# TORlN/HDR-to-SDR

Hardware: AMD Instinct MI355X
Metric: Mpixel/s HDR10->SDR (4K frames) at 1/2/4/8 GPUs; % HBM roofline (higher is better)
Workload: dtype f32

## Files before the change

### hdr-to-sdr_amd/csrc/h2s_tile.h

```cpp
#pragma once
#include <hip/hip_runtime.h>

#include <type_traits>

#include "h2s_device.h"
#include "h2s_dovi.h"

#ifndef H2S_TAGSEL
#define H2S_TAGSEL 1
#endif
#ifndef H2S_EQMAGIC
#define H2S_EQMAGIC 1
#endif
#ifdef H2S_ISA_MARKS
#define H2S_MARK(name)                  \
  do {                                  \
    __builtin_amdgcn_sched_barrier(0);  \
    asm volatile(";@@" name);           \
    __builtin_amdgcn_sched_barrier(0);  \
  } while (0)
#define H2S_MARKV(name, a, b, c)                                  \
  do {                                                            \
    __builtin_amdgcn_sched_barrier(0);                            \
    asm volatile(";@@" name : "+v"(a), "+v"(b), "+v"(c));         \
// ... 577 lines not shown
    asm("v_lshlrev_b16 %0, 1, %1" : "=v"(off) : "v"(qb));
    return *reinterpret_cast<const uint16_t*>(reinterpret_cast<const char*>(eq_lds) + off);
  } else {
    return eq_lds[(int)o.x];
  }
}

constexpr int CBW = 32, CBH = 16;
#ifndef H2S_YST
#define H2S_YST 72
#endif
#ifndef H2S_YST_LP
#define H2S_YST_LP 68
#endif
template <int LP>
constexpr int row_stride() { return LP ? H2S_YST_LP : H2S_YST; }
#ifndef H2S_NT_LOAD
#define H2S_NT_LOAD 2
#endif
#ifndef H2S_NT_STORE
#define H2S_NT_STORE 2
#endif
constexpr int NT = H2S_NT_LOAD, NTS = H2S_NT_STORE;

__device__ __forceinline__ float quad_sum(float v) {
  v += __builtin_bit_cast(float, __builtin_amdgcn_update_dpp(0, __builtin_bit_cast(int, v), 0xB1, 0xF, 0xF, false));
  return v + __builtin_bit_cast(float, __builtin_amdgcn_update_dpp(0, __builtin_bit_cast(int, v), 0x4E, 0xF, 0xF, false));
}

__device__ __forceinline__ void unpack8(const uint4 a, float* o) {
  o[0] = (float)(a.x & 0xffff), o[1] = (float)(a.x >> 16), o[2] = (float)(a.y & 0xffff), o[3] = (float)(a.y >> 16);
  o[4] = (float)(a.z & 0xffff), o[5] = (float)(a.z >> 16), o[6] = (float)(a.w & 0xffff), o[7] = (float)(a.w >> 16);
}

template <class T>
__device__ __forceinline__ T in_vgpr(T x) {
  T y;
  asm volatile("v_mov_b32 %0, %1" : "=v"(y) : "s"(x));
  return y;
}

__device__ __forceinline__ __amdgpu_buffer_rsrc_t plane_rsrc(const uint8_t* base, int bytes) {
  return __builtin_amdgcn_make_buffer_rsrc((void*)base, (short)0, bytes, 0x00020000);
}

template <bool SEMI, int SUB = 0>
struct TileRegs {
  uint4 ya, ua;
  std::conditional_t<SEMI, unsigned, uint16_t> uh;
};
template <bool SEMI>
struct TileRegs<SEMI, 2> {
  uint4 ya, ua, va;
};

struct TileGeo {
  int f, px0, py0, cx0, cy0;
};

__device__ __forceinline__ CurveConsts curve_of(const CurveConsts* frames, int f) {
  typedef __attribute__((address_space(4))) const float cfloat;
  constexpr int n = (int)(sizeof(CurveConsts) / sizeof(float));
  cfloat* src = (cfloat*)frames + __builtin_amdgcn_readfirstlane(f) * n;
  CurveConsts r;
  float* dst = reinterpret_cast<float*>(&r);
#pragma unroll
  for (int i = 0; i < n; i++) dst[i] = src[i];
  return r;
}

__device__ __forceinline__ TileGeo tile_geo(const FastParams& F, unsigned tile) {
  const unsigned bx = tile % F.nbx, bt = tile / F.nbx;
  TileGeo g;
  g.f = (int)(bt / F.nby);
  const int by = (int)(bt % F.nby);
  g.px0 = (int)bx * TBW, g.py0 = by * TBH, g.cx0 = (int)bx * CBW, g.cy0 = by * CBH;
  return g;
}

__device__ __forceinline__ void tile_next(const FastParams& F, TileGeo& g) {
  g.px0 += TBW, g.cx0 += CBW;
  if (g.px0 >= F.W) {
    g.px0 = 0, g.cx0 = 0, g.py0 += TBH, g.cy0 += CBH;
    if (g.py0 >= (int)F.nby * TBH) g.py0 = 0, g.cy0 = 0, g.f++;
  }
}

struct LaneOfs {
  int y, u;
  int sy, sc;
};

template <bool SEMI>
__device__ __forceinline__ LaneOfs lane_ofs(const FastParams& F, int t) {
  LaneOfs L;
  L.y = (t >> 3) * (int)F.in_ls[0] + 16 * (t & 7);
  const int pc = (t >> 7) & 1, tc = t & 127;
  L.u = (tc >> 2) * (int)F.in_ls[1 + pc] + 16 * (tc & 3);
  if (SEMI && F.in_semi) L.u = (t >> 3) * (int)F.in_ls[1] + 16 * (t & 7);
  const int sb = F.out8 ? 8 : 16;
  L.sy = (t >> 3) * (int)F.out_ls[0] + sb * (t & 7);
  const int pl = (t >> 6) & 1, rem = t & 63;
  L.sc = (rem >> 2) * (int)F.out_ls[1 + pl] + sb * (rem & 3);
  if (SEMI && F.out_semi) L.sc = (t >> 3) * (int)F.out_ls[1] + sb * (t & 7);
  return L;
}

template <bool SEMI, int SUB = 0>
__device__ __forceinline__ TileRegs<SEMI, SUB> tile_load(const FastParams& F, const TileGeo& g, int t, const LaneOfs& L) {
  const __amdgpu_buffer_rsrc_t iy = plane_rsrc(F.in[0] + g.f * F.in_fp[0], F.in_bytes[0]);
  const int yr = t >> 3, yc = t & 7;
  TileRegs<SEMI, SUB> r;
  int vy, sy;
  if (g.py0 + TBH <= F.H) {
    vy = L.y, sy = g.py0 * (int)F.in_ls[0] + 2 * g.px0;
  } else {
    vy = (g.py0 + yr < F.H ? g.py0 + yr : F.H - 1) * (int)F.in_ls[0] + 2 * (g.px0 + 8 * yc), sy = 0;
  }
  r.ya = __builtin_bit_cast(uint4, __builtin_amdgcn_raw_buffer_load_b128(iy, vy, sy, NT));
  if constexpr (SUB == 2) {
    const __amdgpu_buffer_rsrc_t iu = plane_rsrc(F.in[1] + g.f * F.in_fp[1], F.in_bytes[1]);
    const __amdgpu_buffer_rsrc_t iv = plane_rsrc(F.in[2] + g.f * F.in_fp[2], F.in_bytes[2]);
    const int lu = (int)F.in_ls[1], lv = (int)F.in_ls[2];
    int vu, vv, su, sv;
    if (g.py0 + TBH <= F.H) {
      vu = yr * lu + 16 * yc, vv = yr * lv + 16 * yc;
      su = g.py0 * lu + 2 * g.px0, sv = g.py0 * lv + 2 * g.px0;
    } else {
      const int row = g.py0 + yr < F.H ? g.py0 + yr : F.H - 1;
      vu = row * lu + 2 * (g.px0 + 8 * yc), vv = row * lv + 2 * (g.px0 + 8 * yc), su = sv = 0;
    }
    r.ua = __builtin_bit_cast(uint4, __builtin_amdgcn_raw_buffer_load_b128(iu, vu, su, NT));
    r.va = __builtin_bit_cast(uint4, __builtin_amdgcn_raw_buffer_load_b128(iv, vv, sv, NT));
    return r;
  } else if constexpr (SUB == 1) {
    const int pc = __builtin_amdgcn_readfirstlane(t >> 7), tc = t & 127;
    const __amdgpu_buffer_rsrc_t ic = plane_rsrc(F.in[1 + pc] + g.f * F.in_fp[1 + pc], F.in_bytes[1 + pc]);
    const int ls = (int)F.in_ls[1 + pc];
    int vc, vh, sc;
    if (g.py0 + TBH <= F.H && g.cx0 + CBW + 1 <= F.icw) {
      vc = L.u, vh = L.u + 16, sc = g.py0 * ls + 2 * g.cx0;
    } else {
      const int clr = tc >> 2, ccx = tc & 3;
      const int row = g.py0 + clr < F.H ? g.py0 + clr : F.H - 1;
      vc = row * ls + 2 * (g.cx0 + 8 * ccx);
      vh = row * ls + 2 * chroma_edge_at(g.cx0 + 8 * ccx + 8, F.icw, F.chroma_edge);
      sc = 0;
    }
    if ((tc & 3) != 3) vh = 0x7FFFFFF0;
    r.ua = __builtin_bit_cast(uint4, __builtin_amdgcn_raw_buffer_load_b128(ic, vc, sc, NT));
    r.uh = __builtin_amdgcn_raw_buffer_load_b16(ic, vh, sc, 0);
    return r;
  } else {
  if (SEMI && F.in_semi) {
    const __amdgpu_buffer_rsrc_t ic = plane_rsrc(F.in[1] + g.f * F.in_fp[1], F.in_bytes[1]);
    const int ls = (int)F.in_ls[1];
    int vc, vh, sc;
    if (g.cy0 >= 1 && g.cy0 + CBH + 1 <= F.ch && g.cx0 + CBW + 1 <= F.cw) {
      vc = L.u, vh = L.u + 16, sc = (g.cy0 - 1) * ls + 4 * g.cx0;
    } else {
      const int clr = t >> 3, ccx = t & 7;
      const int row = chroma_edge_at(g.cy0 - 1 + clr, F.ch, F.chroma_edge);
      vc = row * ls + 4 * (g.cx0 + 4 * ccx);
      vh = row * ls + 4 * chroma_edge_at(g.cx0 + 4 * ccx + 4, F.cw, F.chroma_edge);
      sc = 0;
    }
    if (t >= 144) vc = vh = 0x7FFFFFF0;
    r.ua = __builtin_bit_cast(uint4, __builtin_amdgcn_raw_buffer_load_b128(ic, vc, sc, NT));
    r.uh = __builtin_amdgcn_raw_buffer_load_b32(ic, vh, sc, 0);
    return r;
  }
  const int pc = __builtin_amdgcn_readfirstlane(t >> 7), tc = t & 127;
  const __amdgpu_buffer_rsrc_t ic = plane_rsrc(F.in[1 + pc] + g.f * F.in_fp[1 + pc], F.in_bytes[1 + pc]);
  const int ls = (int)F.in_ls[1 + pc];
  int vc, vh, sc;
  if (g.cy0 >= 1 && g.cy0 + CBH + 1 <= F.ch && g.cx0 + CBW + 1 <= F.cw) {
    vc = L.u, vh = L.u + 16, sc = (g.cy0 - 1) * ls + 2 * g.cx0;
  } else {
    const int clr = tc >> 2, ccx = tc & 3;
    const int row = chroma_edge_at(g.cy0 - 1 + clr, F.ch, F.chroma_edge);
    vc = row * ls + 2 * (g.cx0 + 8 * ccx);
    vh = row * ls + 2 * chroma_edge_at(g.cx0 + 8 * ccx + 8, F.cw, F.chroma_edge);
    sc = 0;
  }
  if (tc >= 72) vc = vh = 0x7FFFFFF0;
  r.ua = __builtin_bit_cast(uint4, __builtin_amdgcn_raw_buffer_load_b128(ic, vc, sc, NT));
  r.uh = __builtin_amdgcn_raw_buffer_load_b16(ic, vh, sc, 0);
  return r;
  }
}

template <int YST>
__device__ __forceinline__ float stage_luma(float* yin, uint4 a, int row, int col8, float ysc, float yoff) {
  float v[8];
  unpack8(a, v);
  float* d = yin + row * YST + 8 * col8;
  const float4 lo = make_float4(fmaf(v[0], ysc, yoff), fmaf(v[1], ysc, yoff), fmaf(v[2], ysc, yoff), fmaf(v[3], ysc, yoff));
  const float4 hi = make_float4(fmaf(v[4], ysc, yoff), fmaf(v[5], ysc, yoff), fmaf(v[6], ysc, yoff), fmaf(v[7], ysc, yoff));
  *reinterpret_cast<float4*>(d) = lo;
  *reinterpret_cast<float4*>(d + 4) = hi;
  return __builtin_fmaxf(__builtin_fmaxf(__builtin_fmaxf(lo.x, lo.y), __builtin_fmaxf(lo.z, lo.w)),
                         __builtin_fmaxf(__builtin_fmaxf(hi.x, hi.y), __builtin_fmaxf(hi.z, hi.w)));
}
template <int HST>
__device__ __forceinline__ float stage_chroma(float* plane, uint4 a, unsigned h, int tt, float cmid) {
  float v[9];
  unpack8(a, v);
  v[8] = (float)h;
#pragma unroll
  for (int k = 0; k < 9; k++) v[k] -= cmid;
  float m = fabsf(v[0]);
#pragma unroll
  for (int k = 1; k < 9; k++) m = __builtin_fmaxf(m, fabsf(v[k]));
  float* d = plane + (tt >> 2) * HST + 16 * (tt & 3);
#pragma unroll
  for (int k = 0; k < 4; k++)
    *reinterpret_cast<float4*>(d + 4 * k) =
        make_float4(v[2 * k] + v[2 * k], v[2 * k] + v[2 * k + 1], v[2 * k + 1] + v[2 * k + 1], v[2 * k + 1] + v[2 * k + 2]);
  return m;
}
template <int HST>
__device__ __forceinline__ float stage_chroma_semi(float* plane_u, float* plane_v, uint4 a, unsigned h, int tt, float cmid) {
  const unsigned w[5] = {a.x, a.y, a.z, a.w, h};
  float u[5], v[5];
#pragma unroll
  for (int k = 0; k < 5; k++) u[k] = (float)(w[k] & 0xffff) - cmid, v[k] = (float)(w[k] >> 16) - cmid;
  float m = __builtin_fmaxf(fabsf(u[0]), fabsf(v[0]));
#pragma unroll
  for (int k = 1; k < 5; k++) m = __builtin_fmaxf(m, __builtin_fmaxf(fabsf(u[k]), fabsf(v[k])));
  const int o = (tt >> 3) * HST + 8 * (tt & 7);
#pragma unroll
  for (int k = 0; k < 2; k++) {
    *reinterpret_cast<float4*>(plane_u + o + 4 * k) =
        make_float4(u[2 * k] + u[2 * k], u[2 * k] + u[2 * k + 1], u[2 * k + 1] + u[2 * k + 1], u[2 * k + 1] + u[2 * k + 2]);
    *reinterpret_cast<float4*>(plane_v + o + 4 * k) =
        make_float4(v[2 * k] + v[2 * k], v[2 * k] + v[2 * k + 1], v[2 * k + 1] + v[2 * k + 1], v[2 * k + 1] + v[2 * k + 2]);
  }
  return m;
}
constexpr int C422_ST = 36;
constexpr int C444_ST = 72;
__device__ __forceinline__ float stage_chroma422(float* plane, uint4 a, unsigned h, int tt, float cmid) {
  float v[9];
  unpack8(a, v);
  v[8] = (float)h;
#pragma unroll
  for (int k = 0; k < 9; k++) v[k] -= cmid;
  float m = fabsf(v[0]);
#pragma unroll
  for (int k = 1; k < 8; k++) m = __builtin_fmaxf(m, fabsf(v[k]));
  float* d = plane + (tt >> 2) * C422_ST + 8 * (tt & 3);
  *reinterpret_cast<float4*>(d) = make_float4(v[0], v[1], v[2], v[3]);
  *reinterpret_cast<float4*>(d + 4) = make_float4(v[4], v[5], v[6], v[7]);
  if ((tt & 3) == 3) d[8] = v[8], m = __builtin_fmaxf(m, fabsf(v[8]));
  return m;
}
__device__ __forceinline__ float stage_chroma444(float* plane_u, float* plane_v, uint4 a, uint4 b, int row, int col8,
                                                 int imid) {
  auto pack = [&](uint4 q, float* plane, float& m) {
    const unsigned w[4] = {q.x, q.y, q.z, q.w};
    unsigned o[4];
#pragma unroll
    for (int k = 0; k < 4; k++) {
      const int lo = (int)(w[k] & 0xffff) - imid, hi = (int)(w[k] >> 16) - imid;
      m = __builtin_fmaxf(m, __builtin_fmaxf(fabsf((float)lo), fabsf((float)hi)));
      o[k] = ((unsigned)lo & 0xffffu) | ((unsigned)hi << 16);
    }
    *reinterpret_cast<uint4*>(reinterpret_cast<int16_t*>(plane) + row * C444_ST + 8 * col8) = make_uint4(o[0], o[1], o[2], o[3]);
  };
  float m = 0.0f;
  pack(a, plane_u, m);
  pack(b, plane_v, m);
  return m;
}
template <int YST>
__device__ __forceinline__ u4v read_luma(const FastParams& F, const float* yin, int r, int c) {
  const unsigned* src = reinterpret_cast<const unsigned*>(yin) + r * YST + 8 * c;
  const uint4 a = *reinterpret_cast<const uint4*>(src), b = *reinterpret_cast<const uint4*>(src + 4);
  if (F.out8)
    return u4v{a.x | (a.y << 8) | (a.z << 16) | (a.w << 24), b.x | (b.y << 8) | (b.z << 16) | (b.w << 24), 0u, 0u};
  return u4v{a.x | (a.y << 16), a.z | (a.w << 16), b.x | (b.y << 16), b.z | (b.w << 16)};
}
__device__ __forceinline__ void put_luma(const FastParams& F, const TileGeo& g, u4v v, int r, int vo, int so) {
  if (g.py0 + r >= F.H) return;
  const __amdgpu_buffer_rsrc_t oy_ = plane_rsrc(F.out[0] + g.f * F.out_fp[0], F.out_bytes[0]);
  so += g.py0 * (int)F.out_ls[0];
  if (F.out8)
    __builtin_amdgcn_raw_buffer_store_b64(u2v{v.x, v.y}, oy_, vo, so + g.px0, NTS);
  else
    __builtin_amdgcn_raw_buffer_store_b128(v, oy_, vo, so + 2 * g.px0, NTS);
}
__device__ __forceinline__ u4v read_chroma(const FastParams& F, const float* csum, int pl, int r, int c) {
  const float4* src = reinterpret_cast<const float4*>(csum + pl * (CBH * CBW) + r * CBW + 8 * c);
  const float4 v0 = src[0], v1 = src[1];
  const float vv[8] = {v0.x, v0.y, v0.z, v0.w, v1.x, v1.y, v1.z, v1.w};
  unsigned code[8];
  if (F.dither) {
#pragma unroll
    for (int k = 0; k < 8; k++) code[k] = (unsigned)(int)(vv[k] + (F.c_bias - 0.5f + dither_off(k, r)));
  } else {
#pragma unroll
    for (int k = 0; k < 8; k++) code[k] = (unsigned)(int)(vv[k] + F.c_bias);
  }
  if (F.rep_rs == 31) {
#pragma unroll
    for (int k = 0; k < 8; k++) code[k] <<= F.shift_out;
  } else {
#pragma unroll
    for (int k = 0; k < 8; k++) code[k] = (code[k] << F.shift_out) | (code[k] >> F.rep_rs);
  }
  if (F.out8)
    return u4v{code[0] | (code[1] << 8) | (code[2] << 16) | (code[3] << 24),
               code[4] | (code[5] << 8) | (code[6] << 16) | (code[7] << 24), 0u, 0u};
  return u4v{code[0] | (code[1] << 16), code[2] | (code[3] << 16), code[4] | (code[5] << 16), code[6] | (code[7] << 16)};
}
__device__ __forceinline__ void put_chroma(const FastParams& F, const TileGeo& g, u4v v, int pl, int r, int vo) {
  if (g.cy0 + r >= F.ch) return;
  const __amdgpu_buffer_rsrc_t oc_ = plane_rsrc(F.out[1 + pl] + g.f * F.out_fp[1 + pl], F.out_bytes[1 + pl]);
  const int so = g.cy0 * (int)F.out_ls[1 + pl];
  if (F.out8)
    __builtin_amdgcn_raw_buffer_store_b64(u2v{v.x, v.y}, oc_, vo, so + g.cx0, NTS);
  else
    __builtin_amdgcn_raw_buffer_store_b128(v, oc_, vo, so + 2 * g.cx0, NTS);
}

__device__ __forceinline__ u4v read_chroma_semi(const FastParams& F, const float* csum, int r, int c) {
  const float4 vu = *reinterpret_cast<const float4*>(csum + r * CBW + 4 * c);
  const float4 vv = *reinterpret_cast<const float4*>(csum + CBH * CBW + r * CBW + 4 * c);
  const float s[8] = {vu.x, vv.x, vu.y, vv.y, vu.z, vv.z, vu.w, vv.w};
  unsigned code[8];
  if (F.dither) {
#pragma unroll
    for (int k = 0; k < 8; k++) code[k] = (unsigned)(int)(s[k] + (F.c_bias - 0.5f + dither_off(4 * (c & 1) + (k >> 1), r)));
  } else {
#pragma unroll
    for (int k = 0; k < 8; k++) code[k] = (unsigned)(int)(s[k] + F.c_bias);
  }
  if (F.rep_rs == 31) {
#pragma unroll
    for (int k = 0; k < 8; k++) code[k] <<= F.shift_out;
  } else {
#pragma unroll
    for (int k = 0; k < 8; k++) code[k] = (code[k] << F.shift_out) | (code[k] >> F.rep_rs);
  }
  if (F.out8)
    return u4v{code[0] | (code[1] << 8) | (code[2] << 16) | (code[3] << 24),
               code[4] | (code[5] << 8) | (code[6] << 16) | (code[7] << 24), 0u, 0u};
  return u4v{(code[0] | (code[1] << 16)) << F.out_sh, (code[2] | (code[3] << 16)) << F.out_sh,
             (code[4] | (code[5] << 16)) << F.out_sh, (code[6] | (code[7] << 16)) << F.out_sh};
}
__device__ __forceinline__ void put_chroma_semi(const FastParams& F, const TileGeo& g, u4v v, int r, int vo) {
  if (g.cy0 + r >= F.ch) return;
  const __amdgpu_buffer_rsrc_t oc_ = plane_rsrc(F.out[1] + g.f * F.out_fp[1], F.out_bytes[1]);
  const int so = g.cy0 * (int)F.out_ls[1];
  if (F.out8)
    __builtin_amdgcn_raw_buffer_store_b64(u2v{v.x, v.y}, oc_, vo, so + 2 * g.cx0, NTS);
  else
    __builtin_amdgcn_raw_buffer_store_b128(v, oc_, vo, so + 4 * g.cx0, NTS);
}

template <int TRC, int TM, int DESAT, int LP, int DBG = 0, bool SEMI = false, int SUB = 0>
#ifndef H2S_TILE_WPE
#define H2S_TILE_WPE 5
#endif
#ifndef H2S_TILE_WPE_LP
#define H2S_TILE_WPE_LP H2S_TILE_WPE
#endif
__global__ __launch_bounds__(256) __attribute__((amdgpu_waves_per_eu(LP ? H2S_TILE_WPE_LP : H2S_TILE_WPE))) void k_tile(
    const FastParams F) {
  static_assert(DBG == 0 || DBG == 1, "the stage is F.dbg_stage, not a template value");
  static_assert(SUB == 0 || SUB == 3 || (LP == 0 && DBG == 0), "4:2:2 / 4:4:4 input: CPU chain product instances only");
  static_assert(SUB != 3 || (DBG == 0 && SEMI), "top-left 4:2:0 input: the SEMI product instances");
  constexpr bool S420 = SUB == 0 || SUB == 3;
  constexpr int YST = row_stride<LP>(), HST = YST;
  static_assert(TBH * C422_ST <= (CBH + 2) * HST && TBH * C444_ST <= 2 * (CBH + 2) * HST, "hrow holds the SUB windows");
  __shared__ float yin[TBH * YST];
  __shared__ float hrow[2][(CBH + 2) * HST];
  __shared__ float csum[2][CBH * CBW];
  __shared__ float4 pq_lds[PQ_NSEG + 1];
  __shared__ float4 pqi_lds[LP ? PQI_NTAB : 1];
  extern __shared__ uint16_t eq_lds[];
  __shared__ int tflag[2];
  __shared__ int offtab[4];
  __shared__ unsigned spread_lds[LP ? 256 : 1];
  constexpr int ESC = TRC == 0 || !LP ? PQ_SEG : 1;

  const int t = threadIdx.x;
  const int lane = t & 63, w = t >> 6;
  const unsigned ntiles = F.nbx * F.nby * F.nframes;
  unsigned tile = (unsigned)xcd_remap(blockIdx.x, gridDim.x) * (unsigned)F.tpb;
  const unsigned tend = tile + (unsigned)F.tpb < ntiles ? tile + (unsigned)F.tpb : ntiles;

  TileGeo geo = tile_geo(F, tile);
  const LaneOfs lofs = lane_ofs<SEMI>(F, t);
  TileRegs<SEMI, SUB> cur = tile_load<SEMI, SUB>(F, geo, t, lofs);
  const __amdgpu_buffer_rsrc_t req = __builtin_amdgcn_make_buffer_rsrc((void*)F.eq_lut, (short)0, 2 * F.eq_n, 0x00020000);
  const unsigned eq0 = __builtin_amdgcn_raw_buffer_load_b16(req, 2 * t, 0, 0);
  float4 pq0 = make_float4(0.0f, 0.0f, 0.0f, 0.0f);
  const bool stage_pq = TRC != 1 || !LP || F.lp_ipt;
  if (stage_pq && t < PQ_NSEG) {
    const __amdgpu_buffer_rsrc_t rpq = __builtin_amdgcn_make_buffer_rsrc((void*)F.pq_tab, (short)0, 16 * PQ_NSEG, 0x00020000);
    pq0 = __builtin_bit_cast(float4, __builtin_amdgcn_raw_buffer_load_b128(rpq, 16 * t, 0, 0));
  }
  const int eq_sh = SEMI ? F.out_sh : 0;
  if (t < F.eq_n) eq_lds[t] = (uint16_t)(((eq0 << F.shift_out) | (eq0 >> F.rep_rs)) << eq_sh);
  for (int i = t + 256; i < F.eq_n; i += 256) {
    const unsigned v = __builtin_amdgcn_raw_buffer_load_b16(req, 2 * i, 0, 0);
    eq_lds[i] = (uint16_t)(((v << F.shift_out) | (v >> F.rep_rs)) << eq_sh);
  }
  if (stage_pq && t < PQ_NSEG)
    pq_lds[t + 1] = (TRC == 0 || LP) && t == 0 ? make_float4(0.0f, 0.0f, 3.40282347e38f, 0.0f) : pq0;
  if (stage_pq && t == 255) pq_lds[0] = make_float4(0.0f, 0.0f, 0.0f, 0.0f);
  if (t < 2) tflag[t] = 0;
  if (t < 3) offtab[t] = t == 0 ? 12 : (t == 1 ? F.og : F.ob);
  if (LP) {
    unsigned x = (unsigned)t;
    x = (x | (x << 8)) & 0x0F00Fu;
    x = (x | (x << 4)) & 0x0C30C3u;
    spread_lds[t] = (x | (x << 2)) & 0x249249u;
  }
  __syncthreads();
  if (LP && (F.lp_ipt || TRC == 2)) {
    const __amdgpu_buffer_rsrc_t rpi = __builtin_amdgcn_make_buffer_rsrc((void*)F.pqi_tab, (short)0, 16 * PQI_NTAB, 0x00020000);
    for (int i = t; i < PQI_NTAB; i += 256)
      pqi_lds[i] = __builtin_bit_cast(float4, __builtin_amdgcn_raw_buffer_load_b128(rpi, 16 * i, 0, 0));
  }

  const int qx = (lane >> 2) & 3, qy = lane >> 4, pxl = lane & 1, pyl = (lane >> 1) & 1;
  const int xl = 16 * w + 2 * qx + pxl, yl = 2 * qy + pyl;
  const float* ybase = yin + yl * YST + xl;
  const float* h0 = hrow[0] + (qy + 1) * HST + xl;
  const float* h1 = hrow[1] + (qy + 1) * HST + xl;
  const int hb = SUB == 3 ? (pyl ? HST : 0) : (pyl ? HST : -HST);
  const float* c0 = hrow[0] + yl * C422_ST + (xl >> 1);
  const float* c1 = hrow[1] + yl * C422_ST + (xl >> 1);
  const int16_t* s0 = reinterpret_cast<const int16_t*>(hrow[0]) + yl * C444_ST + xl;
  const int16_t* s1 = reinterpret_cast<const int16_t*>(hrow[1]) + yl * C444_ST + xl;
  float* csb = csum[0] + qy * CBW + 8 * w + qx;

  const float yoff = in_vgpr(F.y_off_c) * (float)ESC + (ESC == PQ_SEG ? 1.0f : 0.0f);
  const float cmid = in_vgpr(F.c_mid);
  const float a_rv = in_vgpr(F.a_rv[1]) * (float)ESC, a_gv = in_vgpr(F.a_gv[1]) * (float)ESC,
              a_gu = in_vgpr(F.a_gu[1]) * (float)ESC, a_bu = in_vgpr(F.a_bu[1]) * (float)ESC;
  const float stride_g = in_vgpr(F.stride_g), stride_b = in_vgpr(F.stride_b);
  const int og = in_vgpr(F.og), ob = in_vgpr(F.ob), ocr = in_vgpr(F.cr), ocg = in_vgpr(F.cg), ocb = in_vgpr(F.cb);
  const float log2_nm1 = in_vgpr(F.log2_nm1), x_max = in_vgpr(F.x_max);
  const float ysc = in_vgpr(F.ys) * (float)ESC;
  const float ydq = F.dither ? dither_off(xl, yl) - 0.5f : 0.0f;
  const StepK K{a_rv, a_gv, a_gu, a_bu, stride_g, stride_b, og, ob, ocr, ocg, ocb, log2_nm1, x_max,
                TM == 5 && !LP ? in_vgpr(F.hable_kb) : F.hable_kb, F.c111, rintf(1.0f / F.inv_nm1), offtab,
                LP ? in_vgpr(F.lp_k2) : 0.0f, LP ? in_vgpr(F.lp_k2 + 255.0f) : 0.0f, LP ? F.lp_cy + ydq : 0.0f,
                LP ? in_vgpr(F.lp_k1) : 0.0f};
  gu32* lut8v = LP ? in_vgpr64(F.lut8x) : nullptr;
  float qo[4];
#pragma unroll
  for (int i = 0; i < 4; i++)
    qo[i] = LP ? F.lp_qo + (F.lp_dith ? bayer16(xl + 8 * (i & 1), yl + 8 * (i >> 1)) : 0.5f) -
                     (F.lut_off ? 0.0f : F.lp_k2 * F.lp_qs_f)
               : 0.5f;

  auto steps = [&](const TileGeo& g, auto fast) {
    constexpr bool FB = decltype(fast)::value;
    if constexpr (FB) {
      H2S_MARK("body: fast");
    } else {
      H2S_MARK("body: exact-capable");
    }
    CurveConsts cv = F;
    if ((TM == 7 || TM == 8 || LP) && F.cv_frames) cv = curve_of(F.cv_frames, g.f);
    const CDoviRec* const dv =
        TRC == 2 ? (const CDoviRec*)F.dovi + __builtin_amdgcn_readfirstlane(F.dovi_n == 1 ? 0 : F.dovi_f0 + g.f) : nullptr;
    if constexpr (LP && TM == 7) {
      cv.b_e1b = in_vgpr(cv.b_e1b), cv.b_tb = in_vgpr(cv.b_tb), cv.b_c2 = in_vgpr(cv.b_c2);
      cv.b_lc = in_vgpr(cv.b_lc), cv.b_bk_b = in_vgpr(cv.b_bk_b), cv.b_bk_d = in_vgpr(cv.b_bk_d);
    } else if constexpr (LP && TM == 8) {
      cv.sp_qb_u = in_vgpr(cv.sp_qb_u), cv.sp_pb_u = in_vgpr(cv.sp_pb_u);
      cv.sp_srcmax = in_vgpr(cv.sp_srcmax), cv.sp_umax = in_vgpr(cv.sp_umax);
    }
    const __amdgpu_buffer_rsrc_t lut = __builtin_amdgcn_make_buffer_rsrc((void*)F.lut_yuv, (short)0, F.lut_bytes, 0x00020000);
    auto chroma_out = [&](int s, float oyv, float ozv) {
      if (!FB && F.chr444) {
        const int px = g.px0 + xl + 8 * (s & 1), py = g.py0 + yl + 8 * (s >> 1);
        F.chr444[(long long)py * F.chr_w + px] = make_float2(oyv * F.inv_c56, ozv * F.inv_c56);
        return;
      }
      H2S_MARK("S6 chroma quad sums");
      const int oc = 4 * (s >> 1) * CBW + 4 * (s & 1);
      const float su = quad_sum(oyv), sv = quad_sum(ozv);
      csb[oc] = su;
      csb[oc + CBH * CBW] = sv;
    };
    if constexpr (LP && DBG == 0) {
      if (!F.lut_off) {
        unsigned vp = 0;
#pragma unroll
        for (int s = 0; s <= 8; s++) {
          unsigned vn = 0;
          if (s < 8) {
            const int oy = 8 * (s >> 1) * YST + 8 * (s & 1);
            const int oh = 4 * (s >> 1) * HST + 8 * (s & 1);
            H2S_MARK("S0 step: staged Y, vertical chroma");
            const float ybs = ybase[oy];
            const float U = SUB == 3 ? 2.0f * (h0[oh] + h0[oh + hb]) : fmaf(3.0f, h0[oh], h0[oh + hb]);
            const float V = SUB == 3 ? 2.0f * (h1[oh] + h1[oh + hb]) : fmaf(3.0f, h1[oh], h1[oh + hb]);
            float r, gg, bl;
            lin_tone<TRC, TM, DESAT, LP, 0, FB>(F, cv, pq_lds, pqi_lds, K, ybs, U, V, [](float, float, float) {},
                                                 r, gg, bl, dv);
            H2S_MARK("S3 encode");
            vn = lp_table_read(F, K, lut8v, spread_lds, r, gg, bl, qo[s & 3]);
          }
          if (s > 0) {
            const int sp = s - 1;
            const float R8 = (float)(vp & 255u), G8 = (float)((vp >> 8) & 255u), B8 = (float)((vp >> 16) & 255u);
            H2S_MARK("S5 Y'CbCr");
            const f3 o = lp_ycbcr(F, K, R8, G8, B8);
            H2S_MARK("S7 eq");
            reinterpret_cast<unsigned*>(yin)[yl * YST + xl + 8 * (sp >> 1) * YST + 8 * (sp & 1)] = eq_lds[(int)o.x];
            chroma_out(sp, o.y, o.z);
          }
          vp = vn;
        }
        return;
      }
      H2S_MARK("body: lut off");
    }
#pragma unroll
    for (int s = 0; s < 8; s++) {
      const int oy = 8 * (s >> 1) * YST + 8 * (s & 1);
      const int oh = 4 * (s >> 1) * HST + 8 * (s & 1);
      H2S_MARK("S0 step: staged Y, vertical chroma");
      const float ybs = ybase[oy];
      float U, V;
      if constexpr (SUB == 1) {
        const int oc = 8 * (s >> 1) * C422_ST + 4 * (s & 1);
        U = 4.0f * (c0[oc] + c0[oc + pxl]), V = 4.0f * (c1[oc] + c1[oc + pxl]);
      } else if constexpr (SUB == 2) {
        const int oc = 8 * (s >> 1) * C444_ST + 8 * (s & 1);
        U = 8.0f * (float)s0[oc], V = 8.0f * (float)s1[oc];
      } else if constexpr (SUB == 3) {
        U = 2.0f * (h0[oh] + h0[oh + hb]), V = 2.0f * (h1[oh] + h1[oh + hb]);
      } else {
        U = fmaf(3.0f, h0[oh], h0[oh + hb]);
        V = fmaf(3.0f, h1[oh], h1[oh + hb]);
      }
      const long long di = DBG && g.f == 0 && g.py0 + yl + 8 * (s >> 1) < F.H
                               ? (long long)(g.py0 + yl + 8 * (s >> 1)) * F.dbg_w + g.px0 + xl + 8 * (s & 1)
                               : -1;
      float oyv, ozv;
      reinterpret_cast<unsigned*>(yin)[yl * YST + xl + oy] = px_chain<TRC, TM, DESAT, LP, DBG, FB>(
          F, cv, pq_lds, pqi_lds, eq_lds, lut8v, spread_lds, lut, K, ybs, U, V, di, oyv, ozv, LP ? qo[s & 3] : 0.5f, ydq, dv);
      chroma_out(s, oyv, ozv);
    }
  };
  auto mask_in = [&](uint4& a) {
    a.x &= F.in_mask2, a.y &= F.in_mask2, a.z &= F.in_mask2, a.w &= F.in_mask2;
  };
  auto shift_in = [&](uint4& a) { a.x >>= F.in_sh, a.y >>= F.in_sh, a.z >>= F.in_sh, a.w >>= F.in_sh; };

  const int pl = __builtin_amdgcn_readfirstlane(t >> 6) & 1, rem = t & 63;
  const bool cst = t < 128 && !F.chr444;
  for (;;) {
    H2S_MARK("tile: commit, prefetch");
    if (F.in_mask2 != 0xFFFFFFFFu) {
      if constexpr (SEMI && S420) {
        if (F.in_sh) {
          shift_in(cur.ya), shift_in(cur.ua);
          cur.uh >>= F.in_sh;
        }
      }
      mask_in(cur.ya), mask_in(cur.ua);
      if constexpr (SUB == 2) mask_in(cur.va);
      else cur.uh &= F.in_mask2;
    }
    const float my = stage_luma<YST>(yin, cur.ya, t >> 3, t & 7, ysc, yoff);
    float mc = 0.0f;
    if constexpr (SUB == 1) {
      mc = stage_chroma422(hrow[__builtin_amdgcn_readfirstlane(t >> 7)], cur.ua, cur.uh, t & 127, cmid);
    } else if constexpr (SUB == 2) {
      mc = stage_chroma444(hrow[0], hrow[1], cur.ua, cur.va, t >> 3, t & 7, (int)F.c_mid);
    } else if (SEMI && F.in_semi) {
      if (t < 144) mc = stage_chroma_semi<HST>(hrow[0], hrow[1], cur.ua, cur.uh, t, cmid);
    } else if ((t & 127) < 72) {
      mc = stage_chroma<HST>(hrow[__builtin_amdgcn_readfirstlane(t >> 7)], cur.ua, cur.uh, t & 127, cmid);
    }
    const int par = (int)(tile & 1u);
    if ((my > F.safe_y || mc > F.safe_c)) tflag[par] = 1;
    const TileGeo g = geo;
    const bool more = tile + 1 < tend;
    if (more) {
      tile_next(F, geo);
      cur = tile_load<SEMI, SUB>(F, geo, t, lofs);
    }
    __syncthreads();
    const bool fb = __builtin_amdgcn_readfirstlane(tflag[par]) == 0 && !F.chr444;
    if (t == 0) tflag[par ^ 1] = 0;
    if (fb)
      steps(g, std::integral_constant<bool, true>{});
    else
      steps(g, std::integral_constant<bool, false>{});
    H2S_MARK("tile: store");
    __syncthreads();

    put_luma(F, g, read_luma<YST>(F, yin, t >> 3, t & 7), t >> 3, lofs.sy, 0);
    if (cst) {
      if (SEMI && F.out_semi)
        put_chroma_semi(F, g, read_chroma_semi(F, csum[0], t >> 3, t & 7), t >> 3, lofs.sc);
      else
        put_chroma(F, g, read_chroma(F, csum[0], pl, rem >> 2, rem & 3), pl, rem >> 2, lofs.sc);
    }
    if (!more) break;
    ++tile;
    __syncthreads();
  }
}


#define FAST_CASES(X) \
  X(0, 4, 0, 0)       \
  X(0, 4, 1, 0)       \
  X(0, 4, 2, 0)       \
  X(0, 5, 0, 0)       \
  X(0, 5, 1, 0)       \
  X(0, 5, 2, 0)       \
  X(0, 6, 0, 0)       \
  X(0, 6, 1, 0)       \
  X(0, 6, 2, 0)       \
  X(0, 7, 0, 0)       \
  X(0, 8, 0, 0)       \
  X(0, 7, 0, 1)       \
  X(0, 8, 0, 1)       \
  X(0, 4, 0, 1)       \
  X(0, 5, 0, 1)       \
  X(0, 6, 0, 1)       \
  X(1, 4, 0, 0)       \
  X(1, 4, 1, 0)       \
  X(1, 4, 2, 0)       \
  X(1, 5, 0, 0)       \
  X(1, 5, 1, 0)       \
  X(1, 5, 2, 0)       \
  X(1, 6, 0, 0)       \
  X(1, 6, 1, 0)       \
  X(1, 6, 2, 0)       \
  X(1, 7, 0, 0)       \
  X(1, 8, 0, 0)       \
  X(1, 7, 0, 1)       \
  X(1, 8, 0, 1)       \
  X(1, 4, 0, 1)       \
  X(1, 5, 0, 1)       \
  X(1, 6, 0, 1)

template <int DBG, int LPI, bool SEMI = false, int SUB = 0>
hipError_t launch_tile(const FastParams& F, int trc, int tm, int desat, dim3 grid, size_t lds, hipStream_t s) {
#define X(T, M, D, L)                                                                       \
  if constexpr (L == LPI) {                                                                 \
    if (trc == T && tm == M && desat == D) {                                                \
      hipLaunchKernelGGL((k_tile<T, M, D, L, DBG, SEMI, SUB>), grid, dim3(256), lds, s, F); \
      return hipGetLastError();                                                             \
    }                                                                                       \
  }
  FAST_CASES(X)
#undef X
  return hipErrorInvalidValue;
}
template <int DBG, bool SEMI>
hipError_t launch_tile_dv(const FastParams& F, int tm, dim3 grid, size_t lds, hipStream_t s) {
#define X(M)                                                                           \
  if (tm == M) {                                                                       \
    hipLaunchKernelGGL((k_tile<2, M, 0, 1, DBG, SEMI, 0>), grid, dim3(256), lds, s, F); \
    return hipGetLastError();                                                          \
  }
  X(4) X(5) X(6) X(7) X(8)
#undef X
  return hipErrorInvalidValue;
}
#define H2S_TILE_DV_EXTERN(...) \
  extern template hipError_t launch_tile_dv<__VA_ARGS__>(const FastParams&, int, dim3, size_t, hipStream_t);
#define H2S_TILE_DV_INSTANCE(...) \
  template hipError_t launch_tile_dv<__VA_ARGS__>(const FastParams&, int, dim3, size_t, hipStream_t);
#define H2S_TILE_EXTERN(...) \
  extern template hipError_t launch_tile<__VA_ARGS__>(const FastParams&, int, int, int, dim3, size_t, hipStream_t);
#define H2S_TILE_INSTANCE(...) \
  template hipError_t launch_tile<__VA_ARGS__>(const FastParams&, int, int, int, dim3, size_t, hipStream_t);

}
```

Measured before the change: 273,100.

## Stage luma as packed u16 in LDS, merge chroma loads, unify stores, drop barrier

Luma is now staged in LDS as raw 16-bit samples in a bank-conflict-free byte layout instead of pre-scaled floats, and the scale/offset is applied at read time. Peak detection uses packed u16 max. The semi-planar and planar chroma tile loads are merged into one path with a uniform scalar offset and a b32 halo load with the half selected later. Stores are unified into one b128 path that uses DPP lane swaps for 8-bit output and invalid-offset drops instead of branches. The commit stage moves to the loop tail, removing one __syncthreads per tile, and steps for rows beyond the frame bottom are skipped. Together these aim to cut LDS footprint and traffic, per-tile sync and divergence, at the cost of more complex code and some correctness risk at the edges.

```diff
diff --git a/hdr-to-sdr_amd/csrc/h2s_tile.h b/hdr-to-sdr_amd/csrc/h2s_tile.h
--- a/hdr-to-sdr_amd/csrc/h2s_tile.h
+++ b/hdr-to-sdr_amd/csrc/h2s_tile.h
@@ -753,10 +753,11 @@
     r.uh = __builtin_amdgcn_raw_buffer_load_b16(ic, vh, sc, 0);
     return r;
   } else {
-  if (SEMI && F.in_semi) {
-    const __amdgpu_buffer_rsrc_t ic = plane_rsrc(F.in[1] + g.f * F.in_fp[1], F.in_bytes[1]);
+  const bool pair = SEMI && F.in_semi;
+  int pc, vc, vh, sc;
+  if (pair) {
+    pc = 0;
     const int ls = (int)F.in_ls[1];
-    int vc, vh, sc;
     if (g.cy0 >= 1 && g.cy0 + CBH + 1 <= F.ch && g.cx0 + CBW + 1 <= F.cw) {
       vc = L.u, vh = L.u + 16, sc = (g.cy0 - 1) * ls + 4 * g.cx0;
     } else {
@@ -767,41 +768,53 @@
       sc = 0;
     }
     if (t >= 144) vc = vh = 0x7FFFFFF0;
-    r.ua = __builtin_bit_cast(uint4, __builtin_amdgcn_raw_buffer_load_b128(ic, vc, sc, NT));
-    r.uh = __builtin_amdgcn_raw_buffer_load_b32(ic, vh, sc, 0);
-    return r;
-  }
-  const int pc = __builtin_amdgcn_readfirstlane(t >> 7), tc = t & 127;
+  } else {
+    pc = __builtin_amdgcn_readfirstlane(t >> 7);
+    const int tc = t & 127;
+    const int ls = (int)F.in_ls[1 + pc];
+    if (g.cy0 >= 1 && g.cy0 + CBH + 1 <= F.ch && g.cx0 + CBW + 1 <= F.cw) {
+      vc = L.u, vh = L.u + 16, sc = (g.cy0 - 1) * ls + 2 * g.cx0;
+    } else {
+      const int clr = tc >> 2, ccx = tc & 3;
+      const int row = chroma_edge_at(g.cy0 - 1 + clr, F.ch, F.chroma_edge);
+      vc = row * ls + 2 * (g.cx0 + 8 * ccx);
+      vh = row * ls + 2 * chroma_edge_at(g.cx0 + 8 * ccx + 8, F.cw, F.chroma_edge);
+      sc = 0;
+    }
+    if (tc >= 72) vc = vh = 0x7FFFFFF0;
+  }
   const __amdgpu_buffer_rsrc_t ic = plane_rsrc(F.in[1 + pc] + g.f * F.in_fp[1 + pc], F.in_bytes[1 + pc]);
-  const int ls = (int)F.in_ls[1 + pc];
-  int vc, vh, sc;
-  if (g.cy0 >= 1 && g.cy0 + CBH + 1 <= F.ch && g.cx0 + CBW + 1 <= F.cw) {
-    vc = L.u, vh = L.u + 16, sc = (g.cy0 - 1) * ls + 2 * g.cx0;
+  sc = __builtin_amdgcn_readfirstlane(sc);
+  r.ua = __builtin_bit_cast(uint4, __builtin_amdgcn_raw_buffer_load_b128(ic, vc, sc, NT));
+  if constexpr (SEMI) {
+    r.uh = __builtin_amdgcn_raw_buffer_load_b32(ic, vh & ~2, sc, 0);
   } else {
-    const int clr = tc >> 2, ccx = tc & 3;
-    const int row = chroma_edge_at(g.cy0 - 1 + clr, F.ch, F.chroma_edge);
-    vc = row * ls + 2 * (g.cx0 + 8 * ccx);
-    vh = row * ls + 2 * chroma_edge_at(g.cx0 + 8 * ccx + 8, F.cw, F.chroma_edge);
-    sc = 0;
-  }
-  if (tc >= 72) vc = vh = 0x7FFFFFF0;
-  r.ua = __builtin_bit_cast(uint4, __builtin_amdgcn_raw_buffer_load_b128(ic, vc, sc, NT));
-  r.uh = __builtin_amdgcn_raw_buffer_load_b16(ic, vh, sc, 0);
+    r.uh = __builtin_amdgcn_raw_buffer_load_b16(ic, vh, sc, 0);
+  }
   return r;
   }
 }
 
-template <int YST>
-__device__ __forceinline__ float stage_luma(float* yin, uint4 a, int row, int col8, float ysc, float yoff) {
-  float v[8];
-  unpack8(a, v);
-  float* d = yin + row * YST + 8 * col8;
-  const float4 lo = make_float4(fmaf(v[0], ysc, yoff), fmaf(v[1], ysc, yoff), fmaf(v[2], ysc, yoff), fmaf(v[3], ysc, yoff));
-  const float4 hi = make_float4(fmaf(v[4], ysc, yoff), fmaf(v[5], ysc, yoff), fmaf(v[6], ysc, yoff), fmaf(v[7], ysc, yoff));
-  *reinterpret_cast<float4*>(d) = lo;
-  *reinterpret_cast<float4*>(d + 4) = hi;
-  return __builtin_fmaxf(__builtin_fmaxf(__builtin_fmaxf(lo.x, lo.y), __builtin_fmaxf(lo.z, lo.w)),
-                         __builtin_fmaxf(__builtin_fmaxf(hi.x, hi.y), __builtin_fmaxf(hi.z, hi.w)));
+__device__ __forceinline__ unsigned halo_half(const FastParams& F, const TileGeo& g, int t, unsigned hw) {
+  int hs = 0;
+  if (!(g.cy0 >= 1 && g.cy0 + CBH + 1 <= F.ch && g.cx0 + CBW + 1 <= F.cw))
+    hs = (chroma_edge_at(g.cx0 + 8 * (t & 3) + 8, F.cw, F.chroma_edge) & 1) << 4;
+  return (hw >> hs) & 0xffffu;
+}
+
+constexpr int YROW = 144;
+constexpr int luma_at(int x, int y) { return y * YROW + 2 * x; }
+static_assert(YROW % 16 == 0 && luma_at(8, 0) == 16, "a chunk of 8 samples is one aligned 16-byte slot");
+static_assert(luma_at(0, 1) >= luma_at(TBW - 1, 0) + 2, "the rows' slots are disjoint");
+static_assert((luma_at(0, 1) / 4) % 32 == 4 && luma_at(7, 0) / 4 == 3, "a step's 8 rows x 4 dwords cover the 32 banks once");
+constexpr int YIN_BYTES = luma_at(0, TBH);
+typedef unsigned short us2v __attribute__((ext_vector_type(2)));
+__device__ __forceinline__ float stage_luma(unsigned char* yin, uint4 a, int row, int col8, float ysc, float yoff) {
+  *reinterpret_cast<uint4*>(yin + luma_at(8 * col8, row)) = a;
+  const us2v m = __builtin_elementwise_max(
+      __builtin_elementwise_max(__builtin_bit_cast(us2v, a.x), __builtin_bit_cast(us2v, a.y)),
+      __builtin_elementwise_max(__builtin_bit_cast(us2v, a.z), __builtin_bit_cast(us2v, a.w)));
+  return fmaf((float)(m.x > m.y ? m.x : m.y), ysc, yoff);
 }
 template <int HST>
 __device__ __forceinline__ float stage_chroma(float* plane, uint4 a, unsigned h, int tt, float cmid) {
@@ -874,22 +887,25 @@
   pack(b, plane_v, m);
   return m;
 }
-template <int YST>
-__device__ __forceinline__ u4v read_luma(const FastParams& F, const float* yin, int r, int c) {
-  const unsigned* src = reinterpret_cast<const unsigned*>(yin) + r * YST + 8 * c;
-  const uint4 a = *reinterpret_cast<const uint4*>(src), b = *reinterpret_cast<const uint4*>(src + 4);
+__device__ __forceinline__ u4v read_luma(const FastParams& F, const unsigned char* yin, int r, int c) {
+  const uint4 a = *reinterpret_cast<const uint4*>(yin + luma_at(8 * c, r));
   if (F.out8)
-    return u4v{a.x | (a.y << 8) | (a.z << 16) | (a.w << 24), b.x | (b.y << 8) | (b.z << 16) | (b.w << 24), 0u, 0u};
-  return u4v{a.x | (a.y << 16), a.z | (a.w << 16), b.x | (b.y << 16), b.z | (b.w << 16)};
-}
-__device__ __forceinline__ void put_luma(const FastParams& F, const TileGeo& g, u4v v, int r, int vo, int so) {
-  if (g.py0 + r >= F.H) return;
+    return u4v{__builtin_amdgcn_perm(a.y, a.x, 0x06040200u), __builtin_amdgcn_perm(a.w, a.z, 0x06040200u), 0u, 0u};
+  return u4v{a.x, a.y, a.z, a.w};
+}
+constexpr int ST_DROP = (int)0x80000000u;
+__device__ __forceinline__ void tile_store(const FastParams& F, u4v v, __amdgpu_buffer_rsrc_t rs, int vo, int so, int t) {
+  if (F.out8) {
+    v.z = (unsigned)__builtin_amdgcn_update_dpp(0, (int)v.x, 0xB1, 0xF, 0xF, false);
+    v.w = (unsigned)__builtin_amdgcn_update_dpp(0, (int)v.y, 0xB1, 0xF, 0xF, false);
+    if (t & 1) vo = ST_DROP;
+  }
+  __builtin_amdgcn_raw_buffer_store_b128(v, rs, vo, so, NTS);
+}
+__device__ __forceinline__ void put_luma(const FastParams& F, const TileGeo& g, u4v v, int r, int vo, int t) {
+  if (g.py0 + r >= F.H) vo = ST_DROP;
   const __amdgpu_buffer_rsrc_t oy_ = plane_rsrc(F.out[0] + g.f * F.out_fp[0], F.out_bytes[0]);
-  so += g.py0 * (int)F.out_ls[0];
-  if (F.out8)
-    __builtin_amdgcn_raw_buffer_store_b64(u2v{v.x, v.y}, oy_, vo, so + g.px0, NTS);
-  else
-    __builtin_amdgcn_raw_buffer_store_b128(v, oy_, vo, so + 2 * g.px0, NTS);
+  tile_store(F, v, oy_, vo, g.py0 * (int)F.out_ls[0] + (F.out8 ? g.px0 : 2 * g.px0), t);
 }
 __device__ __forceinline__ u4v read_chroma(const FastParams& F, const float* csum, int pl, int r, int c) {
   const float4* src = reinterpret_cast<const float4*>(csum + pl * (CBH * CBW) + r * CBW + 8 * c);
@@ -915,14 +931,9 @@
                code[4] | (code[5] << 8) | (code[6] << 16) | (code[7] << 24), 0u, 0u};
   return u4v{code[0] | (code[1] << 16), code[2] | (code[3] << 16), code[4] | (code[5] << 16), code[6] | (code[7] << 16)};
 }
-__device__ __forceinline__ void put_chroma(const FastParams& F, const TileGeo& g, u4v v, int pl, int r, int vo) {
-  if (g.cy0 + r >= F.ch) return;
+__device__ __forceinline__ void put_chroma(const FastParams& F, const TileGeo& g, u4v v, int pl, bool semi, int vo, int t) {
   const __amdgpu_buffer_rsrc_t oc_ = plane_rsrc(F.out[1 + pl] + g.f * F.out_fp[1 + pl], F.out_bytes[1 + pl]);
-  const int so = g.cy0 * (int)F.out_ls[1 + pl];
-  if (F.out8)
-    __builtin_amdgcn_raw_buffer_store_b64(u2v{v.x, v.y}, oc_, vo, so + g.cx0, NTS);
-  else
-    __builtin_amdgcn_raw_buffer_store_b128(v, oc_, vo, so + 2 * g.cx0, NTS);
+  tile_store(F, v, oc_, vo, g.cy0 * (int)F.out_ls[1 + pl] + ((F.out8 ? g.cx0 : 2 * g.cx0) << (semi ? 1 : 0)), t);
 }
 
 __device__ __forceinline__ u4v read_chroma_semi(const FastParams& F, const float* csum, int r, int c) {
@@ -950,16 +961,6 @@
   return u4v{(code[0] | (code[1] << 16)) << F.out_sh, (code[2] | (code[3] << 16)) << F.out_sh,
              (code[4] | (code[5] << 16)) << F.out_sh, (code[6] | (code[7] << 16)) << F.out_sh};
 }
-__device__ __forceinline__ void put_chroma_semi(const FastParams& F, const TileGeo& g, u4v v, int r, int vo) {
-  if (g.cy0 + r >= F.ch) return;
-  const __amdgpu_buffer_rsrc_t oc_ = plane_rsrc(F.out[1] + g.f * F.out_fp[1], F.out_bytes[1]);
-  const int so = g.cy0 * (int)F.out_ls[1];
-  if (F.out8)
-    __builtin_amdgcn_raw_buffer_store_b64(u2v{v.x, v.y}, oc_, vo, so + 2 * g.cx0, NTS);
-  else
-    __builtin_amdgcn_raw_buffer_store_b128(v, oc_, vo, so + 4 * g.cx0, NTS);
-}
-
 template <int TRC, int TM, int DESAT, int LP, int DBG = 0, bool SEMI = false, int SUB = 0>
 #ifndef H2S_TILE_WPE
 #define H2S_TILE_WPE 5
@@ -975,7 +976,7 @@
   constexpr bool S420 = SUB == 0 || SUB == 3;
   constexpr int YST = row_stride<LP>(), HST = YST;
   static_assert(TBH * C422_ST <= (CBH + 2) * HST && TBH * C444_ST <= 2 * (CBH + 2) * HST, "hrow holds the SUB windows");
-  __shared__ float yin[TBH * YST];
+  __shared__ __attribute__((aligned(16))) unsigned char yin[YIN_BYTES];
   __shared__ float hrow[2][(CBH + 2) * HST];
   __shared__ float csum[2][CBH * CBW];
   __shared__ float4 pq_lds[PQ_NSEG + 1];
@@ -1029,7 +1030,7 @@
 
   const int qx = (lane >> 2) & 3, qy = lane >> 4, pxl = lane & 1, pyl = (lane >> 1) & 1;
   const int xl = 16 * w + 2 * qx + pxl, yl = 2 * qy + pyl;
-  const float* ybase = yin + yl * YST + xl;
+  uint16_t* ybase = reinterpret_cast<uint16_t*>(yin + luma_at(xl, yl));
   const float* h0 = hrow[0] + (qy + 1) * HST + xl;
   const float* h1 = hrow[1] + (qy + 1) * HST + xl;
   const int hb = SUB == 3 ? (pyl ? HST : 0) : (pyl ? HST : -HST);
@@ -1062,6 +1063,7 @@
 
   auto steps = [&](const TileGeo& g, auto fast) {
     constexpr bool FB = decltype(fast)::value;
+    constexpr int YR2 = YROW / 2;
     if constexpr (FB) {
       H2S_MARK("body: fast");
     } else {
@@ -1079,6 +1081,7 @@
       cv.sp_srcmax = in_vgpr(cv.sp_srcmax), cv.sp_umax = in_vgpr(cv.sp_umax);
     }
     const __amdgpu_buffer_rsrc_t lut = __builtin_amdgcn_make_buffer_rsrc((void*)F.lut_yuv, (short)0, F.lut_bytes, 0x00020000);
+    const int live = !FB && DBG == 0 && !F.chr444 ? F.H - g.py0 : TBH;
     auto chroma_out = [&](int s, float oyv, float ozv) {
       if (!FB && F.chr444) {
         const int px = g.px0 + xl + 8 * (s & 1), py = g.py0 + yl + 8 * (s >> 1);
@@ -1097,11 +1100,11 @@
 #pragma unroll
         for (int s = 0; s <= 8; s++) {
           unsigned vn = 0;
-          if (s < 8) {
-            const int oy = 8 * (s >> 1) * YST + 8 * (s & 1);
+          if (s < 8 && (FB || 8 * (s >> 1) < live)) {
+            const int oy = 8 * (s >> 1) * YR2 + 8 * (s & 1);
             const int oh = 4 * (s >> 1) * HST + 8 * (s & 1);
             H2S_MARK("S0 step: staged Y, vertical chroma");
-            const float ybs = ybase[oy];
+            const float ybs = fmaf((float)ybase[oy], ysc, yoff);
             const float U = SUB == 3 ? 2.0f * (h0[oh] + h0[oh + hb]) : fmaf(3.0f, h0[oh], h0[oh + hb]);
             const float V = SUB == 3 ? 2.0f * (h1[oh] + h1[oh + hb]) : fmaf(3.0f, h1[oh], h1[oh + hb]);
             float r, gg, bl;
@@ -1110,13 +1113,13 @@
             H2S_MARK("S3 encode");
             vn = lp_table_read(F, K, lut8v, spread_lds, r, gg, bl, qo[s & 3]);
           }
-          if (s > 0) {
+          if (s > 0 && (FB || 8 * ((s - 1) >> 1) < live)) {
             const int sp = s - 1;
             const float R8 = (float)(vp & 255u), G8 = (float)((vp >> 8) & 255u), B8 = (float)((vp >> 16) & 255u);
             H2S_MARK("S5 Y'CbCr");
             const f3 o = lp_ycbcr(F, K, R8, G8, B8);
             H2S_MARK("S7 eq");
-            reinterpret_cast<unsigned*>(yin)[yl * YST + xl + 8 * (sp >> 1) * YST + 8 * (sp & 1)] = eq_lds[(int)o.x];
+            ybase[8 * (sp >> 1) * YR2 + 8 * (sp & 1)] = eq_lds[(int)o.x];
             chroma_out(sp, o.y, o.z);
           }
           vp = vn;
@@ -1127,10 +1130,11 @@
     }
 #pragma unroll
     for (int s = 0; s < 8; s++) {
-      const int oy = 8 * (s >> 1) * YST + 8 * (s & 1);
+      if (!FB && (s & 1) == 0 && 8 * (s >> 1) >= live) break;
+      const int oy = 8 * (s >> 1) * YR2 + 8 * (s & 1);
       const int oh = 4 * (s >> 1) * HST + 8 * (s & 1);
       H2S_MARK("S0 step: staged Y, vertical chroma");
-      const float ybs = ybase[oy];
+      const float ybs = fmaf((float)ybase[oy], ysc, yoff);
       float U, V;
       if constexpr (SUB == 1) {
         const int oc = 8 * (s >> 1) * C422_ST + 4 * (s & 1);
@@ -1148,7 +1152,7 @@
                                ? (long long)(g.py0 + yl + 8 * (s >> 1)) * F.dbg_w + g.px0 + xl + 8 * (s & 1)
                                : -1;
       float oyv, ozv;
-      reinterpret_cast<unsigned*>(yin)[yl * YST + xl + oy] = px_chain<TRC, TM, DESAT, LP, DBG, FB>(
+      ybase[oy] = (uint16_t)px_chain<TRC, TM, DESAT, LP, DBG, FB>(
           F, cv, pq_lds, pqi_lds, eq_lds, lut8v, spread_lds, lut, K, ybs, U, V, di, oyv, ozv, LP ? qo[s & 3] : 0.5f, ydq, dv);
       chroma_out(s, oyv, ozv);
     }
@@ -1160,8 +1164,11 @@
 
   const int pl = __builtin_amdgcn_readfirstlane(t >> 6) & 1, rem = t & 63;
   const bool cst = t < 128 && !F.chr444;
-  for (;;) {
-    H2S_MARK("tile: commit, prefetch");
+  auto commit = [&](unsigned ti) {
+    H2S_MARK("tile: commit");
+    if constexpr (SEMI && S420) {
+      if (!F.in_semi) cur.uh = halo_half(F, geo, t, cur.uh);
+    }
     if (F.in_mask2 != 0xFFFFFFFFu) {
       if constexpr (SEMI && S420) {
         if (F.in_sh) {
@@ -1173,7 +1180,7 @@
       if constexpr (SUB == 2) mask_in(cur.va);
       else cur.uh &= F.in_mask2;
     }
-    const float my = stage_luma<YST>(yin, cur.ya, t >> 3, t & 7, ysc, yoff);
+    const float my = stage_luma(yin, cur.ya, t >> 3, t & 7, ysc, yoff);
     float mc = 0.0f;
     if constexpr (SUB == 1) {
       mc = stage_chroma422(hrow[__builtin_amdgcn_readfirstlane(t >> 7)], cur.ua, cur.uh, t & 127, cmid);
@@ -1184,8 +1191,14 @@
     } else if ((t & 127) < 72) {
       mc = stage_chroma<HST>(hrow[__builtin_amdgcn_readfirstlane(t >> 7)], cur.ua, cur.uh, t & 127, cmid);
     }
+    if constexpr (SUB == 2) asm volatile("" ::"v"(cur.ua.w), "v"(cur.va.w));
+    else asm volatile("" ::"v"(cur.ua.w), "v"(cur.uh));
+    if ((my > F.safe_y || mc > F.safe_c)) tflag[ti & 1u] = 1;
+  };
+  commit(tile);
+  for (;;) {
+    H2S_MARK("tile: prefetch");
     const int par = (int)(tile & 1u);
-    if ((my > F.safe_y || mc > F.safe_c)) tflag[par] = 1;
     const TileGeo g = geo;
     const bool more = tile + 1 < tend;
     if (more) {
@@ -1193,7 +1206,7 @@
       cur = tile_load<SEMI, SUB>(F, geo, t, lofs);
     }
     __syncthreads();
-    const bool fb = __builtin_amdgcn_readfirstlane(tflag[par]) == 0 && !F.chr444;
+    const bool fb = __builtin_amdgcn_readfirstlane(tflag[par]) == 0 && !F.chr444 && !(DBG == 0 && g.py0 + TBH > F.H);
     if (t == 0) tflag[par ^ 1] = 0;
     if (fb)
       steps(g, std::integral_constant<bool, true>{});
@@ -1202,16 +1215,18 @@
     H2S_MARK("tile: store");
     __syncthreads();
 
-    put_luma(F, g, read_luma<YST>(F, yin, t >> 3, t & 7), t >> 3, lofs.sy, 0);
+    put_luma(F, g, read_luma(F, yin, t >> 3, t & 7), t >> 3, lofs.sy, t);
+    const bool osemi = SEMI && F.out_semi;
+    u4v cv{0u, 0u, 0u, 0u};
+    int cvo = ST_DROP;
     if (cst) {
-      if (SEMI && F.out_semi)
-        put_chroma_semi(F, g, read_chroma_semi(F, csum[0], t >> 3, t & 7), t >> 3, lofs.sc);
-      else
-        put_chroma(F, g, read_chroma(F, csum[0], pl, rem >> 2, rem & 3), pl, rem >> 2, lofs.sc);
-    }
+      const int cr = osemi ? t >> 3 : rem >> 2;
+      cv = osemi ? read_chroma_semi(F, csum[0], cr, t & 7) : read_chroma(F, csum[0], pl, cr, rem & 3);
+      if (g.cy0 + cr < F.ch) cvo = lofs.sc;
+    }
+    put_chroma(F, g, cv, osemi ? 0 : pl, osemi, cvo, t);
     if (!more) break;
-    ++tile;
-    __syncthreads();
+    commit(++tile);
   }
 }
 
```

Measured after the change: 277,400, median of 6. +1.6%, better.
